# BUTSpeechFIT/VBx

Measured on NVIDIA H100. Metric: x-vectors/sec through 10 VB-HMM EM iters, higher is better.
Workload: dtype f32

## Files before the change

include/vbx_b200.h:

```cpp
#ifndef VBX_B200_H
#define VBX_B200_H

#include <stddef.h>
#include <stdint.h>

#ifdef __cplusplus
extern "C" {
#endif

typedef struct vbx_handle_s *vbx_handle_t;

enum vbx_status {
    VBX_OK = 0,
    VBX_ERR_ARG = -1,
    VBX_ERR_CUDA = -2,
    VBX_ERR_STATE = -3,
    VBX_ERR_NO_DEVICE = -4
};

enum vbx_flag {
    VBX_FLAG_NONFINITE = 1,
    VBX_FLAG_ELBO_DECREASED = 2,
    VBX_FLAG_CONVERGED = 4
};
// ... 161 lines not shown

int vbx_stream_window(vbx_handle_t h, int32_t n, int32_t C, int32_t R, int32_t S_max, int32_t S, const int32_t *slot,
                      const int64_t *blk_off, const int64_t *win_off, const int32_t *blk_lab, const int32_t *n_clusters,
                      const float *blk_fea, double smoothing, const float *ctx_fea, const int32_t *ctx_lab,
                      const int64_t *count, const int32_t *K, const double *n_hist, const double *F_hist, float *fea_out,
                      float *gamma_out, float *pi_out, int32_t *n_states_out, double *prior_n_out, double *prior_F_out,
                      void *stream);
int vbx_stream_commit(vbx_handle_t h, int32_t n, int32_t C, int32_t R, int32_t S_max, const int32_t *slot,
                      const int64_t *blk_off, const int64_t *win_off, const float *blk_fea, const int32_t *first,
                      float *ctx_fea, int32_t *ctx_lab, int64_t *count, int32_t *K, double *n_hist, double *F_hist,
                      int32_t *labels_out, void *stream);

int vbx_stream_enroll_workspace_bytes(vbx_handle_t h, int32_t n, int64_t M, int64_t E, int32_t max_k,
                                      size_t *bytes_out);
int vbx_stream_enroll(vbx_handle_t h, int32_t n, int32_t slots, int32_t C, int32_t R, int32_t S_max,
                      const int32_t *slot, const int64_t *cand_off, const int32_t *cand_k, const float *Phi, double Fa,
                      double Fb, const float *ctx_fea, const int32_t *ctx_lab, const int64_t *count, double *n_hist,
                      double *F_hist, int32_t *named, const double *n_enroll, const double *F_enroll, int64_t E,
                      double threshold, int32_t prior, void *workspace, size_t workspace_bytes, int32_t *assign_out,
                      double *best_llr_out, double *llr_out, double *n_out, double *F_out, void *stream);

int64_t vbx_launch_count(vbx_handle_t h);

enum vbx_kernel_class {
    VBX_K_PROJECT = 0,
    VBX_K_PREPARE = 1,
    VBX_K_RUN_INIT = 2,
    VBX_K_MSTEP = 3,
    VBX_K_SPEAKER_MODEL = 4,
    VBX_K_LOGLIK = 5,
    VBX_K_FWDBWD = 6,
    VBX_K_EXACT64 = 7,
    VBX_K_EM_CONTRACT = 8,
    VBX_N_KERNEL_CLASSES = 9
};
int vbx_get_timings(vbx_handle_t h, double *ms_out, int64_t *count_out, int32_t reset);

#ifdef __cplusplus
}
#endif
#endif
```

vbx_b200/_lib.py:

```python
import ctypes
import os

_HERE = os.path.dirname(os.path.abspath(__file__))
LIB_PATH = os.environ.get('VBX_B200_LIB', os.path.join(_HERE, 'libvbx_b200.so'))

EXPORTS = ['vbx_version', 'vbx_padded_states', 'vbx_padded_states_wide', 'vbx_create', 'vbx_destroy', 'vbx_last_error',
           'vbx_set_option', 'vbx_plan', 'vbx_bind_workspace', 'vbx_prepare_scale',
           'vbx_prepare_project', 'vbx_prepare_xvectors', 'vbx_run', 'vbx_run_per_recording', 'vbx_hard_labels', 'vbx_hard_labels_keep', 'vbx_ahc_workspace_bytes', 'vbx_ahc', 'vbx_launch_count', 'vbx_get_timings', 'vbx_f64_workspace_bytes',
           'vbx_run_f64', 'vbx_plan_f64', 'vbx_forward_backward', 'vbx_attach_comm', 'vbx_elbo_trace', 'vbx_get_gsum',
           'vbx_score', 'vbx_score_overlap', 'vbx_score_jer', 'vbx_link_batch_workspace_bytes', 'vbx_link_batch',
           'vbx_enroll_batch_workspace_bytes', 'vbx_enroll_batch', 'vbx_cohort_stats_batch_workspace_bytes',
           'vbx_cohort_stats_batch', 'vbx_init_turns', 'vbx_combine_workspace_bytes', 'vbx_combine',
           'vbx_init_random', 'vbx_run_prior', 'vbx_run_f64_prior', 'vbx_class_scatter_workspace_bytes',
           'vbx_class_scatter', 'vbx_stream_window', 'vbx_stream_commit', 'vbx_verify_score_workspace_bytes',
           'vbx_verify_score', 'vbx_verify_metrics_workspace_bytes', 'vbx_verify_metrics',
           'vbx_verify_calibrate_workspace_bytes', 'vbx_verify_calibrate', 'vbx_stream_enroll_workspace_bytes',
           'vbx_stream_enroll']

FLAG_NONFINITE, FLAG_ELBO_DECREASED, FLAG_CONVERGED = 1, 2, 4
SCORE_BAD_LABEL, SCORE_BAD_REGION, SCORE_BAD_RECORDING = 1, 2, 4
COMBINE_BAD_LABEL, COMBINE_TOO_MANY_LABELS = 1, 2
LINK_MAX_SPEAKERS = 1 << 29
KERNEL_CLASSES = ['project', 'prepare', 'run_init', 'mstep_partial', 'speaker_model', 'loglik', 'forward_backward', 'exact64', 'em_contract']


class VbxError(RuntimeError):
    pass


_lib = None


def load():
    global _lib
    if _lib is not None:
        return _lib
    if not os.path.exists(LIB_PATH):
        raise VbxError(f'{LIB_PATH} is missing - run `python -c "import __graft_entry__ as g; g.build()"` '
                       '(there is no CPU fallback for the VB-HMM path)')
    lib = ctypes.CDLL(LIB_PATH)
# ... 20 lines not shown
    lib.vbx_bind_workspace.argtypes = [vp, vp, ctypes.c_size_t]
    lib.vbx_prepare_scale.restype = ctypes.c_int
    lib.vbx_prepare_scale.argtypes = [vp, vp, vp, vp, vp]
    lib.vbx_prepare_project.restype = ctypes.c_int
    lib.vbx_prepare_project.argtypes = [vp, vp, i32, vp, vp, vp, vp]
    lib.vbx_ahc_workspace_bytes.restype = ctypes.c_int
    lib.vbx_ahc_workspace_bytes.argtypes = [vp, ctypes.POINTER(ctypes.c_size_t)]
    lib.vbx_ahc.restype = ctypes.c_int
    lib.vbx_ahc.argtypes = [vp, vp, i32, i32, vp, ctypes.c_size_t, vp, vp, vp]
    lib.vbx_hard_labels.restype = ctypes.c_int
    lib.vbx_hard_labels.argtypes = [vp, vp, vp, vp, vp, vp]
    lib.vbx_hard_labels_keep.restype = ctypes.c_int
    lib.vbx_hard_labels_keep.argtypes = [vp, vp, vp, vp, vp, vp, vp, vp]
    lib.vbx_prepare_xvectors.restype = ctypes.c_int
    lib.vbx_prepare_xvectors.argtypes = [vp, vp, i32, vp, vp, vp, vp, vp, vp, vp, vp, vp]
    lib.vbx_run.restype = ctypes.c_int
    lib.vbx_run.argtypes = [vp, vp, vp, vp, vp, vp, dbl, dbl, dbl, i32, dbl, vp, vp, i32, vp, vp, vp, vp]
    lib.vbx_run_per_recording.restype = ctypes.c_int
    lib.vbx_run_per_recording.argtypes = [vp, vp, vp, vp, vp, vp, vp, vp, vp, i32, dbl, vp, vp, i32, vp, vp, vp, vp]
    lib.vbx_run_prior.restype = ctypes.c_int
    lib.vbx_run_prior.argtypes = [vp, vp, vp, vp, vp, vp, vp, vp, vp, i32, dbl, vp, vp, i32, vp, vp, vp, vp, vp, vp]
    lib.vbx_launch_count.restype = i64
    lib.vbx_launch_count.argtypes = [vp]
    lib.vbx_f64_workspace_bytes.restype = ctypes.c_int
    lib.vbx_f64_workspace_bytes.argtypes = [vp, ctypes.POINTER(ctypes.c_size_t)]
    lib.vbx_run_f64.restype = ctypes.c_int
    lib.vbx_run_f64.argtypes = [vp, vp, ctypes.c_size_t, vp, vp, vp, vp, vp, dbl, dbl, dbl, i32, dbl, vp, vp, i32, vp, vp, vp, vp]
    lib.vbx_run_f64_prior.restype = ctypes.c_int
    lib.vbx_run_f64_prior.argtypes = [vp, vp, ctypes.c_size_t, vp, vp, vp, vp, vp, dbl, dbl, dbl, i32, dbl, vp, vp, i32, vp, vp,
                                      vp, vp, vp, vp]
    lib.vbx_forward_backward.restype = ctypes.c_int
    lib.vbx_forward_backward.argtypes = [vp, vp, vp, vp, i32, i32, vp, vp, vp, vp, vp]
    lib.vbx_attach_comm.restype = ctypes.c_int
    lib.vbx_attach_comm.argtypes = [vp, vp, i32, ctypes.c_char_p]
    lib.vbx_elbo_trace.restype = ctypes.c_int
    lib.vbx_elbo_trace.argtypes = [vp, vp, i32, vp, vp]
    lib.vbx_get_gsum.restype = ctypes.c_int
    lib.vbx_get_gsum.argtypes = [vp, vp, vp]
    lib.vbx_score.restype = ctypes.c_int
    lib.vbx_score.argtypes = [vp, i32, vp, vp, vp, vp, vp, vp, vp, vp, vp, i32, vp, vp, vp, vp, vp, i64, vp, vp, vp, vp, vp]
    lib.vbx_score_overlap.restype = ctypes.c_int
    lib.vbx_score_overlap.argtypes = [vp, i32, vp, vp, vp, vp, vp, vp, vp, vp, vp, vp, i32, vp, vp, vp, vp, vp, vp, i64, vp, vp,
                                      vp, vp, vp]
    lib.vbx_score_jer.restype = ctypes.c_int
    lib.vbx_score_jer.argtypes = [vp, i32, vp, vp, vp, vp, vp, vp, vp, vp, vp, vp, i32, vp, vp, vp, vp, vp, vp, i64, vp, vp, vp,
                                  vp, vp, vp, vp]
# ... 67 lines not shown
```

vbx_b200/batch.py:

```python
import ctypes
import os

import numpy as np
import torch

from . import _lib
from ._lib import VbxError


def _ptr(t):
    return ctypes.c_void_p(t.data_ptr()) if t is not None else None


class VbxBatch:

    def __init__(self, lengths, R, n_states, device=None, allocate=True, exact_stop=True, fb_split=0, S_pad=None, f64_only=False):
        if not torch.cuda.is_available():
            raise VbxError('vbx_b200 needs a CUDA device (H100, sm_90); there is no CPU path')
        self.lib = _lib.load()
        self.device = torch.device('cuda', torch.cuda.current_device()) if device is None else torch.device(device)
        if self.device.index is None:
            self.device = torch.device('cuda', torch.cuda.current_device())
        lengths = np.asarray(lengths, dtype=np.int64).reshape(-1)
        self.B = int(lengths.shape[0])
# ... 139 lines not shown
        self._check(self.lib.vbx_init_turns(self._h, *(_ptr(a) for a in arrays), _ptr(gamma), _ptr(pi),
                                            int(dt == torch.float64), self._stream()))

    def init_random(self, rec_keys, seeds, gamma, pi):
        dt = gamma.dtype
        for t, shape, name in ((gamma, (self.N, self.S), 'gamma'), (pi, (self.B, self.S), 'pi')):
            if not (isinstance(t, torch.Tensor) and t.is_cuda and t.dtype == dt and t.is_contiguous()
                    and dt in (torch.float32, torch.float64) and tuple(t.shape) == shape):
                raise ValueError(f'{name}: expected a contiguous float32 or float64 CUDA tensor of shape {shape}, '
                                 'gamma and pi of one type')
        words = []
        for vals, name in ((rec_keys, 'rec_keys'), (seeds, 'seeds')):
            vals = list(vals)
            if len(vals) != self.B or not all(isinstance(v, (int, np.integer)) and 0 <= int(v) < 1 << 64 for v in vals):
                raise ValueError(f'{name}: expected {self.B} integers in [0, 2**64)')
            a = np.array([int(v) for v in vals], dtype=np.uint64).view(np.int64)
            words.append(torch.from_numpy(a).to(self.device))
        self._check(self.lib.vbx_init_random(self._h, _ptr(words[0]), _ptr(words[1]), _ptr(self.n_states), _ptr(gamma),
                                             _ptr(pi), int(dt == torch.float64), self._stream()))

    @property
    def launches(self):
        return int(self.lib.vbx_launch_count(self._h))

    def timings(self, reset=True):
        n = len(_lib.KERNEL_CLASSES)
        ms = (ctypes.c_double * n)()
        cnt = (ctypes.c_int64 * n)()
        self._check(self.lib.vbx_get_timings(self._h, ms, cnt, int(reset)))
        return {k: (ms[i], cnt[i]) for i, k in enumerate(_lib.KERNEL_CLASSES)}

    def _stream(self):
        return ctypes.c_void_p(torch.cuda.current_stream(self.device).cuda_stream)

    def _f32(self, t, shape, name, need_workspace=True):
        if need_workspace and self.workspace is None:
            raise VbxError('no workspace bound (VbxBatch(..., allocate=False) needs bind())')
        if not (isinstance(t, torch.Tensor) and t.is_cuda and t.dtype == torch.float32 and t.is_contiguous()):
            raise ValueError(f'{name}: expected a contiguous float32 CUDA tensor')
        if tuple(t.shape) != tuple(shape):
            raise ValueError(f'{name}: expected shape {tuple(shape)}, got {tuple(t.shape)}')
        return t

    def prepare_scale(self, fea, Phi, out=None):
        self._f32(fea, (self.N, self.R), 'fea')
        self._f32(Phi, (self.R,), 'Phi')
# ... 423 lines not shown
```

vbx_b200/csrc/vbx_capi.cu:

```cuda
#include <dlfcn.h>
#include <nvtx3/nvToolsExt.h>

#include <algorithm>
#include <cmath>
#include <cstdio>
#include <cstring>
#include <initializer_list>
#include <map>
#include <mutex>
#include <numeric>
#include <string>
#include <utility>
#include <vector>

#include "../../include/vbx_b200.h"
#include "vbx_internal.cuh"

bool vbx::allow_dynamic_smem(const void *kernel, int bytes) {
    int dev = 0;
    if (cudaGetDevice(&dev) != cudaSuccess) return false;
    static std::mutex mu;
    static std::map<std::pair<const void *, int>, int> allowed;
    std::lock_guard<std::mutex> lock(mu);
    int &have = allowed[{kernel, dev}];
    if (have >= bytes) return true;
    if (cudaFuncSetAttribute(kernel, cudaFuncAttributeMaxDynamicSharedMemorySize, bytes) != cudaSuccess) return false;
    have = bytes;
    return true;
}

struct vbx_handle_s {
    int device = 0;
    int sms = 0;
    std::string err;
    vbx::Plan plan;
    vbx::Workspace ws;
    bool planned = false, bound = false, prepared = false;
    bool f64_only = false;
    size_t ws_need = 0;
    void *plan_mem = nullptr;
    int opt_fb_spl = 0;
    int opt_fb_classic = 0;
    int opt_fb_ring = 1;
    int opt_projection = 0;
    int opt_timing = 0;
    int opt_gemm = 0;
    int opt_debug_sync = 0;
    int opt_fb_split = 0;
    int opt_exact_stop = 1;
    int64_t launches = 0;
    cudaStream_t hi_stream = nullptr;
    cudaEvent_t ev_fork = nullptr, ev_join = nullptr;
    int opt_graph = 0;
    cudaStream_t graph_stream = nullptr;
    cudaEvent_t ev_g0 = nullptr, ev_g1 = nullptr;
    cudaGraphExec_t graph_exec = nullptr;
    uint64_t graph_key = 0, seen_key = 0;
    int64_t graph_launches = 0;
    bool graph_broken = false;
    void *nccl_comm = nullptr;
    int nccl_ranks = 1;
// ... 355 lines not shown
    pl.R = R;
    pl.S = S;
    pl.exact = h->opt_exact_stop;
    pl.split = split ? 1 : 0;
    pl.em_cluster = vbx::em_contract_cluster(S, R, maxT, split);
    pl.n_frames = n_rec ? offsets_host[n_rec] : 0;
    pl.n_ltiles = (int32_t)lrec.size();
    pl.n_mtiles = (int32_t)mrec.size();
    pl.max_T = maxT;
    pl.offsets = reinterpret_cast<const int64_t *>(base + o_off);
    pl.order = reinterpret_cast<const int32_t *>(base + o_ord);
    pl.ltile_rec = reinterpret_cast<const int32_t *>(base + o_lrec);
    pl.ltile_f0 = reinterpret_cast<const int64_t *>(base + o_lf0);
    pl.mtile_rec = reinterpret_cast<const int32_t *>(base + o_mrec);
    pl.mtile_f0 = reinterpret_cast<const int64_t *>(base + o_mf0);
    pl.mtile_begin = reinterpret_cast<const int32_t *>(base + o_mb);
    pl.n_lrec = (int32_t)lrec_list.size();
    pl.n_lchunks = (int32_t)lchunk_rec.size();
    pl.lrec_list = reinterpret_cast<const int32_t *>(base + o_ll);
    pl.lrec_first = reinterpret_cast<const int32_t *>(base + o_lf);
    pl.lrec_nchunks = reinterpret_cast<const int32_t *>(base + o_ln);
    pl.lchunk_rec = reinterpret_cast<const int32_t *>(base + o_lcr);
    pl.lchunk_idx = reinterpret_cast<const int32_t *>(base + o_lci);
    h->ws_need = carve(pl, nullptr, nullptr);
    h->offsets_host.assign(offsets_host, offsets_host + (n_rec ? n_rec + 1 : 0));
    if (n_rec == 0) h->offsets_host.assign(1, 0);
    h->ahc_need = vbx::ahc_workspace_bytes(h->offsets_host.data(), n_rec, &h->ahc_d_off);
    h->planned = true;
    if (workspace_bytes_out) *workspace_bytes_out = h->ws_need;
    return VBX_OK;
}

int vbx_plan_f64(vbx_handle_t h, const int64_t *offsets_host, int32_t n_rec, int32_t R, int32_t S) {
    if (!h || !offsets_host || n_rec < 0) return fail(h, VBX_ERR_ARG, "vbx_plan_f64: null argument");
    if (R < 1 || S < 1 || S > 3600) return fail(h, VBX_ERR_ARG, "vbx_plan_f64: need R >= 1 and 1 <= S <= 3600");
    if (n_rec > 0 && offsets_host[0] != 0) return fail(h, VBX_ERR_ARG, "vbx_plan_f64: offsets[0] must be 0");
    for (int b = 0; b < n_rec; ++b) {
        const int64_t T = offsets_host[b + 1] - offsets_host[b];
        if (T < 0 || T > (int64_t)1 << 30) return fail(h, VBX_ERR_ARG, "vbx_plan_f64: bad recording length");
    }
    DeviceGuard guard(h->device);
    if (guard.err != cudaSuccess) return cuda_fail(h, guard.err, "cudaSetDevice");
    if (h->plan_mem) {
        cudaFree(h->plan_mem);
        h->plan_mem = nullptr;
    }
    h->planned = h->bound = h->prepared = false;
    cudaError_t e = cudaMalloc(&h->plan_mem, sizeof(int64_t) * (n_rec + 1));
    if (e != cudaSuccess) return cuda_fail(h, e, "cudaMalloc(plan)");
    e = cudaMemcpy(h->plan_mem, offsets_host, sizeof(int64_t) * (n_rec + 1), cudaMemcpyHostToDevice);
    if (e != cudaSuccess) return cuda_fail(h, e, "cudaMemcpy(plan)");
    h->plan = vbx::Plan();
    h->plan.n_rec = n_rec;
    h->plan.R = R;
    h->plan.S = S;
    h->plan.n_frames = n_rec ? offsets_host[n_rec] : 0;
    h->plan.offsets = static_cast<const int64_t *>(h->plan_mem);
    h->offsets_host.assign(offsets_host, offsets_host + n_rec + 1);
    h->ahc_need = 0;
    h->planned = true;
    h->f64_only = true;
    return VBX_OK;
}

int vbx_bind_workspace(vbx_handle_t h, void *workspace, size_t bytes) {
    if (!h) return VBX_ERR_ARG;
    if (!h->planned) return fail(h, VBX_ERR_STATE, "vbx_bind_workspace: call vbx_plan first");
    if (h->f64_only) return fail(h, VBX_ERR_STATE, "vbx_bind_workspace: the plan came from vbx_plan_f64 (float64 entry points only)");
    if (!workspace || bytes < h->ws_need) return fail(h, VBX_ERR_STATE, "vbx_bind_workspace: workspace too small");
    const size_t mis = reinterpret_cast<uintptr_t>(workspace) & 255;
    char *base = static_cast<char *>(workspace) + (mis ? 256 - mis : 0);
    carve(h->plan, base, &h->ws);
    drop_graph(h);
    h->bound = true;
    h->prepared = false;
// ... 185 lines not shown
                    rc = counted(h, h->opt_gemm ? vbx::launch_mstep_partial(pl, h->ws, rho, gamma_io, st)
                                                : vbx::launch_mstep_mma(pl, h->ws, rho, gamma_io, st), "mstep_partial");
                }
                if (rc) return rc;
                {
                    Timed t(h, st, VBX_K_SPEAKER_MODEL);
                    rc = counted(h, vbx::launch_speaker_model(pl, h->ws, Phi, n_states, alpha_io, invL_io, given, st, prior_n,
                                                              prior_F), "speaker_model");
                }
                if (rc) return rc;
                {
                    Timed t(h, st, VBX_K_LOGLIK);
                    rc = counted(h, h->opt_gemm ? vbx::launch_loglik(pl, h->ws, rho, pi_io, n_states, st) : vbx::launch_loglik_mma(pl, h->ws, rho, pi_io, n_states, st), "loglik");
                }
                if (rc) return rc;
            }
            if (fb_hi) {
                cudaEventRecord(h->ev_fork, st);
                cudaStreamWaitEvent(h->hi_stream, h->ev_fork, 0);
            }
            {
                cudaStream_t fs = fb_hi ? h->hi_stream : st;
                Timed t(h, fs, VBX_K_FWDBWD);
                rc = counted(h, vbx::launch_forward_backward(pl, h->ws, rp, gamma_io, pi_io, n_states, Li_out, n_iters_out, flags_out, it, h->opt_fb_spl, h->opt_fb_classic, h->opt_fb_ring, fs), "forward_backward");
            }
            if (fb_hi) {
                cudaEventRecord(h->ev_join, h->hi_stream);
                cudaStreamWaitEvent(st, h->ev_join, 0);
            }
            if (rc) return rc;
        }
        if (rp.hybrid && it > 0) {
            Timed t(h, st, VBX_K_EXACT64);
            rc = counted(h, vbx::launch_exact64_round(pl, h->ws, rp, rho, Phi, gamma_io, pi_io, n_states, alpha_io, invL_io, Li_out,
                                                      n_iters_out, flags_out, st, prior_n, prior_F), "exact64");
            if (rc) return rc;
        }
    }
    return VBX_OK;
    };

    cudaStream_t user = (cudaStream_t)stream;
    const bool want_graph = (h->opt_graph == 1 || (h->opt_graph == 0 && pl.split)) && !h->opt_timing && !h->opt_debug_sync &&
                            !h->graph_broken;
    if (!want_graph) return enqueue(user);
    uint64_t key = 1469598103934665603ull;
    auto mix = [&](uint64_t v) { key = (key ^ v) * 1099511628211ull; };
// ... 872 lines not shown
    if (rc) return rc;
    if (h->nccl_comm && h->nccl_ranks > 1) {
        const int nrc = h->nccl_allreduce(trace_out, trace_out, (size_t)2 * max_iters,  8,  0, h->nccl_comm, st);
        if (nrc != 0) return fail(h, VBX_ERR_CUDA, "vbx_elbo_trace: ncclAllReduce failed with code " + std::to_string(nrc));
    }
    return VBX_OK;
}

int vbx_get_gsum(vbx_handle_t h, double *gsum_out, void *stream) {
    if (!h) return VBX_ERR_ARG;
    if (!h->planned || !h->bound || !h->prepared) return fail(h, VBX_ERR_STATE, "vbx_get_gsum: call vbx_prepare_* first");
    if (h->plan.n_rec == 0) return VBX_OK;
    if (!gsum_out) return fail(h, VBX_ERR_ARG, "vbx_get_gsum: null pointer");
    DeviceGuard guard(h->device);
    if (guard.err != cudaSuccess) return cuda_fail(h, guard.err, "cudaSetDevice");
    const cudaError_t e = cudaMemcpyAsync(gsum_out, h->ws.gsum, sizeof(double) * h->plan.n_rec, cudaMemcpyDeviceToDevice,
                                          (cudaStream_t)stream);
    if (e != cudaSuccess) return cuda_fail(h, e, "vbx_get_gsum");
    return VBX_OK;
}

int64_t vbx_launch_count(vbx_handle_t h) { return h ? h->launches : -1; }

int vbx_get_timings(vbx_handle_t h, double *ms_out, int64_t *count_out, int32_t reset) {
    if (!h) return VBX_ERR_ARG;
    DeviceGuard guard(h->device);
    for (size_t i = 0; i + 1 < h->ev_used; i += 2) {
        cudaError_t e = cudaEventSynchronize(h->ev_pool[i + 1]);
        if (e != cudaSuccess) return cuda_fail(h, e, "cudaEventSynchronize");
        float ms = 0.f;
        e = cudaEventElapsedTime(&ms, h->ev_pool[i], h->ev_pool[i + 1]);
        if (e != cudaSuccess) return cuda_fail(h, e, "cudaEventElapsedTime");
        const int cls = h->ev_class[i / 2];
        h->t_ms[cls] += ms;
        h->t_cnt[cls] += 1;
    }
    h->ev_used = 0;
    h->ev_class.clear();
    for (int c = 0; c < VBX_N_KERNEL_CLASSES; ++c) {
        if (ms_out) ms_out[c] = h->t_ms[c];
        if (count_out) count_out[c] = h->t_cnt[c];
        if (reset) {
            h->t_ms[c] = 0.0;
            h->t_cnt[c] = 0;
        }
    }
// ... 5 lines not shown
```

vbx_b200/csrc/vbx_em_contract.cu:

```cuda
#include <cooperative_groups.h>
#include <math_constants.h>

#include "vbx_internal.cuh"

namespace cg = cooperative_groups;

namespace vbx {

namespace {
constexpr int kSlots = 4;
constexpr int kRows = 8;
constexpr int kHeld = kMTile / kRows / kSlots;
constexpr int kBars = 4;
constexpr int kLD = kMaxR + 4;
constexpr int kRedBytes = 16 * kLD * 4;
constexpr int kRhoBytes = kHeld * kRows * kMaxR * 4;
constexpr int kSmemBytes = kRhoBytes + kRedBytes + (kBars + 1) * 8;

__device__ __forceinline__ uint32_t cluster_addr(uint32_t a, uint32_t rank) {
    uint32_t r;
    asm volatile("mapa.shared::cluster.u32 %0, %1, %2;" : "=r"(r) : "r"(a), "r"(rank));
    return r;
}
__device__ __forceinline__ void st_async(uint32_t addr, float v, uint32_t bar) {
// ... 318 lines not shown
static int em_contract_cluster_t() {
    cudaLaunchConfig_t cfg = {};
    cfg.gridDim = dim3(CL);
    cfg.blockDim = dim3(128);
    cfg.dynamicSmemBytes = kSmemBytes;
    int n = 0;
    if (!allow_dynamic_smem(em_contract_kernel<S_PAD, CL>, kSmemBytes) ||
        cudaOccupancyMaxActiveClusters(&n, em_contract_kernel<S_PAD, CL>, &cfg) != cudaSuccess)
        return (void)cudaGetLastError(), 0;
    return n >= 1 ? CL : 0;
}

int em_contract_cluster(int S, int R, int64_t max_T, bool split) {
    if (split || R != kMaxR || max_T > 2 * kMTile) return 0;
    const bool two = max_T > kMTile;
    switch (S) {
        case 4: return two ? em_contract_cluster_t<4, 8>() : em_contract_cluster_t<4, 4>();
        case 8: return two ? em_contract_cluster_t<8, 8>() : em_contract_cluster_t<8, 4>();
        case 16: return two ? em_contract_cluster_t<16, 8>() : em_contract_cluster_t<16, 4>();
        default: return 0;
    }
}

int launch_em_contract(const Plan &pl, const Workspace &ws, const float *rho, const float *gamma, const float *Phi,
                       const int32_t *n_states, float *alpha_io, float *invL_io, cudaStream_t st) {
    if (pl.n_rec == 0) return 0;
    const int CL = pl.em_cluster;
#define VBX_EMC(S_, CL_)                                                                                                 \
    em_contract_kernel<S_, CL_><<<pl.n_rec * CL_, 128, kSmemBytes, st>>>(pl, ws, rho, gamma, Phi, n_states, alpha_io, invL_io)
    switch (pl.S * 16 + CL) {
        case 4 * 16 + 4: VBX_EMC(4, 4); break;
        case 4 * 16 + 8: VBX_EMC(4, 8); break;
        case 8 * 16 + 4: VBX_EMC(8, 4); break;
        case 8 * 16 + 8: VBX_EMC(8, 8); break;
        case 16 * 16 + 4: VBX_EMC(16, 4); break;
        case 16 * 16 + 8: VBX_EMC(16, 8); break;
        default: return -1;
    }
#undef VBX_EMC
    return cudaGetLastError() == cudaSuccess ? 1 : -1;
}

}
```

vbx_b200/csrc/vbx_internal.cuh:

```cuda
#pragma once
#include <cuda_runtime.h>
#include <stdint.h>

#include <cfloat>
#include <string>
#include <vector>

#define VBX_EPS_TR 1e-8f

namespace vbx {

constexpr int kLTile = 64;
constexpr int kMTile = 512;
constexpr int kLongT = 4096;
constexpr int kChunk = 256;
constexpr int kMaxR = 128;
constexpr int kMaxS = 64;
constexpr int kMaxSWide = 128;
constexpr int kTcMaxD = 2048;

__host__ __device__ inline size_t al(size_t v) { return (v + 255) & ~(size_t)255; }

struct Plan {
    int32_t n_rec = 0, R = 0, S = 0;
// ... 55 lines not shown
    float *scratch = nullptr;
    float *ahat = nullptr, *bhat = nullptr;
    float *socc = nullptr, *sent = nullptr;
    float *tc_scratch = nullptr;
    float *fa_u = nullptr, *fa_lam = nullptr, *fa_exp = nullptr, *astart = nullptr;
    float *bb_v = nullptr, *bb_mu = nullptr, *bb_exp = nullptr, *beta = nullptr;
    float *occp = nullptr, *entp = nullptr;
    RecParams *hp = nullptr;
};

struct RunParams {
    double epsilon;
    int32_t max_iters;
    int32_t hybrid, warm;
};
constexpr double kStopNoiseC = 2.0;
constexpr double kStopGuardMult = 16.0;

bool allow_dynamic_smem(const void *kernel, int bytes);
template <class... Args>
bool allow_dynamic_smem(void (*kernel)(Args...), int bytes) {
    return allow_dynamic_smem(reinterpret_cast<const void *>(kernel), bytes);
}

#ifdef __CUDACC__
template <int N>
struct Vec {
    float v[N];
};
template <int N>
__device__ __forceinline__ Vec<N> ld_vec(const float *p);
template <>
__device__ __forceinline__ Vec<1> ld_vec<1>(const float *p) {
    Vec<1> r;
    r.v[0] = *p;
    return r;
}
template <>
__device__ __forceinline__ Vec<2> ld_vec<2>(const float *p) {
    float2 t = *reinterpret_cast<const float2 *>(p);
    Vec<2> r;
    r.v[0] = t.x;
    r.v[1] = t.y;
    return r;
}
template <>
// ... 194 lines not shown

__device__ __forceinline__ double as_norm(double l, const double *mean_i, const double *std_i, int64_t i,
                                          const double *mean_j, const double *std_j, int64_t j) {
    return 0.5 * ((l - mean_i[i]) / std_i[i] + (l - mean_j[j]) / std_j[j]);
}

#endif

int launch_prepare_scale(const Plan &pl, const Workspace &ws, const float *fea, const float *Phi, float *rho,
                         cudaStream_t st);
int launch_project_ffma(const Plan &pl, const float *X, int D, const float *V, float *rho, cudaStream_t st);
int launch_g_from_rho(const Plan &pl, const Workspace &ws, const float *rho, const float *Phi, cudaStream_t st);
int launch_run_init(const Plan &pl, const Workspace &ws, const float *gamma, const int32_t *n_states, double *Li,
                    int32_t *n_iters, int32_t *flags, int max_iters, double Fa, double Fb, double loopP,
                    const double *Fa_v, const double *Fb_v, const double *loopP_v, cudaStream_t st);
int launch_mstep_partial(const Plan &pl, const Workspace &ws, const float *rho, const float *gamma, cudaStream_t st);
int launch_speaker_model(const Plan &pl, const Workspace &ws, const float *Phi,
                         const int32_t *n_states, float *alpha_io, float *invL_io, bool from_given,
                         cudaStream_t st, const double *prior_n = nullptr, const double *prior_F = nullptr);
int launch_loglik(const Plan &pl, const Workspace &ws, const float *rho, const float *pi, const int32_t *n_states,
                  cudaStream_t st);
int launch_forward_backward(const Plan &pl, const Workspace &ws, const RunParams &rp, float *gamma, float *pi,
                            const int32_t *n_states, double *Li, int32_t *n_iters, int32_t *flags, int iter,
                            int spl, int classic, int ring, cudaStream_t st);
int launch_elbo_trace(const Plan &pl, const double *Li, int max_iters, double *out, cudaStream_t st);
int launch_forward_backward_split(const Plan &pl, const Workspace &ws, const RunParams &rp, float *gamma, float *pi,
                                  const int32_t *n_states, int spl, cudaStream_t st);
int launch_forward_backward_long(const Plan &pl, const Workspace &ws, const RunParams &rp, float *gamma, float *pi,
                                 const int32_t *n_states, cudaStream_t st);
int launch_mstep_mma(const Plan &pl, const Workspace &ws, const float *rho, const float *gamma, cudaStream_t st);
int launch_loglik_mma(const Plan &pl, const Workspace &ws, const float *rho, const float *pi, const int32_t *n_states,
                      cudaStream_t st);
int em_contract_cluster(int S, int R, int64_t max_T, bool split);
int launch_em_contract(const Plan &pl, const Workspace &ws, const float *rho, const float *gamma, const float *Phi,
                       const int32_t *n_states, float *alpha_io, float *invL_io, cudaStream_t st);
int launch_snapshot(const Plan &pl, const Workspace &ws, const float *gamma, const float *pi, int iter, cudaStream_t st);
int launch_exact64_round(const Plan &pl, const Workspace &ws, const RunParams &rp, const float *rho, const float *Phi,
                         float *gamma, float *pi, const int32_t *n_states, float *alpha_io, float *invL_io, double *Li,
                         int32_t *n_iters, int32_t *flags, cudaStream_t st, const double *prior_n = nullptr,
                         const double *prior_F = nullptr);
size_t f64_workspace_bytes(const Plan &pl);
int launch_run_f64(const Plan &pl, void *workspace, const double *fea, const double *Phi, double *gamma, double *pi,
                   const int32_t *n_states, double Fa, double Fb, double loopP, int max_iters, double epsilon,
                   double *alpha_io, double *invL_io, int warm, double *Li, int32_t *n_iters, int32_t *flags,
                   cudaStream_t st, const double *prior_n = nullptr, const double *prior_F = nullptr);
int launch_hard_labels(const Plan &pl, const float *gamma, const int32_t *n_states, int32_t *first, int32_t *second,
                       cudaStream_t st);
int launch_hard_labels_keep(const Plan &pl, const float *gamma, const int32_t *n_states, const int32_t *keep,
                            int32_t *first, int32_t *second, double *mass, cudaStream_t st);
int launch_init_turns(const Plan &pl, const int64_t *seg, const int64_t *spk_off, const int64_t *turn_off,
                      const int64_t *turn_lo, const int64_t *turn_hi, const int64_t *turn_cum, const double *smoothing,
                      void *gamma, void *pi, bool f64, cudaStream_t st);
int launch_init_random(const Plan &pl, const uint64_t *rec_key, const uint64_t *seed, const int32_t *n_states,
                       void *gamma, void *pi, bool f64, cudaStream_t st);
int launch_fb_dense(const double *lls, const double *tr, const double *ip, int T, int S, double *post, double *tll,
                    double *lfw, double *lbw, cudaStream_t st);
// ... 116 lines not shown
```

vbx_b200/csrc/vbx_kernels.cu:

```cuda
#include <math_constants.h>

#include "vbx_internal.cuh"

namespace vbx {

__device__ __forceinline__ void cp_async16(void *smem, const void *gmem) {
    unsigned s = static_cast<unsigned>(__cvta_generic_to_shared(smem));
    asm volatile("cp.async.cg.shared.global [%0], [%1], 16;\n" ::"r"(s), "l"(gmem));
}
__device__ __forceinline__ void cp_async_wait_all() {
    asm volatile("cp.async.commit_group;\n" ::);
    asm volatile("cp.async.wait_group 0;\n" ::: "memory");
}

template <int LANES>
__device__ __forceinline__ float group_max(float v) {
#pragma unroll
    for (int off = LANES / 2; off > 0; off >>= 1) v = fmaxf(v, __shfl_xor_sync(0xffffffffu, v, off));
    return v;
}
__device__ __forceinline__ double warp_sum_d(double v) {
#pragma unroll
    for (int off = 16; off > 0; off >>= 1) v += __shfl_xor_sync(0xffffffffu, v, off);
    return v;
// ... 1512 lines not shown
            else
                bstage(u, st, rb, true);
        }
    }

    double pn[SPL];
    float loc = 0.f;
#pragma unroll
    for (int k = 0; k < SPL; ++k) {
        pn[k] = (double)g0[k] + (double)Q * (double)pi[k] * enter[k];
        loc += (float)pn[k];
    }
    const float tot = group_sum<LPR>(loc);
    if (live) {
#pragma unroll
        for (int k = 0; k < SPL; ++k) {
            const int s = l * SPL + k;
            pi_io[(int64_t)rec * S_PAD + s] = (float)(pn[k] / (double)tot);
            ws.occ[(int64_t)rec * S_PAD + s] = (float)occ[k];
        }
    }
}

constexpr int64_t kRingMaxT = 2048;

template <int S_PAD, int SPL>
static int launch_fb_t(const Plan &pl, const Workspace &ws, const RunParams &rp, float *gamma, float *pi,
                       const int32_t *n_states, bool classic, bool ring, cudaStream_t st) {
    constexpr int RPW = 32 / (S_PAD / SPL);
    const int warps = (pl.n_rec + RPW - 1) / RPW;
    const int blocks = (warps + 3) / 4;
    if (classic) {
        forward_backward_kernel<S_PAD, SPL><<<blocks, 128, 0, st>>>(pl, ws, rp, gamma, pi, n_states);
    } else if (ring && pl.max_T <= kRingMaxT) {
        constexpr int smem = FbRing<S_PAD, SPL>::kSmemBytes;
        if (!allow_dynamic_smem(forward_backward_ring_kernel<S_PAD, SPL>, smem)) return -1;
        forward_backward_ring_kernel<S_PAD, SPL><<<blocks, 128, smem, st>>>(pl, ws, rp, gamma, pi, n_states);
    } else {
        forward_backward_la_kernel<S_PAD, SPL><<<blocks, 128, 0, st>>>(pl, ws, rp, gamma, pi, n_states);
    }
    return cudaGetLastError() == cudaSuccess ? 1 : -1;
}

__global__ void __launch_bounds__(128) elbo_kernel(Plan pl, Workspace ws, RunParams rp, double *Li, int32_t *n_iters,
                                                   int32_t *flags, int iter) {
    const int rec = blockIdx.x;
    if (!ws.active[rec]) return;
    const int tid = threadIdx.x, lane = tid & 31, warp = tid >> 5;
    const int64_t f0 = pl.offsets[rec];
    const int T = (int)(pl.offsets[rec + 1] - f0);
    const float *rs = ws.rsigma + f0;
    const float *mx = ws.rowmax + f0;
    double acc = 0.0;
    for (int t = tid; t < T; t += 128) acc += (double)mx[t] - log((double)rs[t]);
    acc = warp_sum_d(acc);
    __shared__ double part[4];
// ... 49 lines not shown
    __shared__ double ss[256], cs[256];
    ss[tid] = s;
    cs[tid] = c;
    __syncthreads();
    for (int off = 128; off > 0; off >>= 1) {
        if (tid < off) {
            ss[tid] += ss[tid + off];
            cs[tid] += cs[tid + off];
        }
        __syncthreads();
    }
    if (tid == 0) {
        out[it] = ss[0];
        out[max_iters + it] = cs[0];
    }
}
int launch_elbo_trace(const Plan &pl, const double *Li, int max_iters, double *out, cudaStream_t st) {
    elbo_trace_kernel<<<max_iters, 256, 0, st>>>(pl.n_rec, Li, max_iters, out);
    return cudaGetLastError() == cudaSuccess ? 1 : -1;
}

int launch_forward_backward(const Plan &pl, const Workspace &ws, const RunParams &rp, float *gamma, float *pi,
                            const int32_t *n_states, double *Li, int32_t *n_iters, int32_t *flags, int iter,
                            int spl, int classic, int ring, cudaStream_t st) {
    if (pl.n_rec == 0) return 0;
    if (pl.split) {
        const int rs = launch_forward_backward_split(pl, ws, rp, gamma, pi, n_states, spl, st);
        if (rs < 0) return rs;
        elbo_kernel<<<pl.n_rec, 128, 0, st>>>(pl, ws, rp, Li, n_iters, flags, iter);
        return cudaGetLastError() == cudaSuccess ? rs + 1 : -1;
    }
    int rc = -1;
#define VBX_FB(S_, L_) rc = launch_fb_t<S_, L_>(pl, ws, rp, gamma, pi, n_states, classic != 0, ring != 0, st)
    const int S = pl.S;
    if (spl == 0) spl = (S >= 16) ? 2 : 1;
    if (S == 64 && spl < 2) spl = 2;
    if (spl > S) spl = S;
    switch (S) {
        case 4:
            if (spl == 1) VBX_FB(4, 1);
            else if (spl == 2) VBX_FB(4, 2);
            else VBX_FB(4, 4);
            break;
        case 8:
            if (spl == 1) VBX_FB(8, 1);
            else if (spl == 2) VBX_FB(8, 2);
            else VBX_FB(8, 4);
            break;
        case 16:
            if (spl == 1) VBX_FB(16, 1);
            else if (spl == 2) VBX_FB(16, 2);
            else VBX_FB(16, 4);
            break;
        case 32:
            if (spl == 1) VBX_FB(32, 1);
            else if (spl == 2) VBX_FB(32, 2);
// ... 18 lines not shown
```

Measured before the change: 201.9 million.

## Add shared-memory-free forward-backward kernel that co-resides with EM contraction

Adds a forward-backward variant that keeps its checkpoints in the gamma output buffer instead of dynamic shared memory. It is chosen when an occupancy check shows one of its CTAs fits on an SM beside the resident em_contract CTAs, so the two stages can overlap across streams. It also sets the max-shared carveout preference on the new kernel and on the ELBO kernel. The cost is more global-memory traffic for checkpoint reloads, plus a host-side occupancy heuristic that may misjudge residency.

```diff
diff --git a/include/vbx_b200.h b/include/vbx_b200.h
--- a/include/vbx_b200.h
+++ b/include/vbx_b200.h
@@ -207,6 +207,8 @@
 
 int64_t vbx_launch_count(vbx_handle_t h);
 
+int vbx_plan_property(vbx_handle_t h, const char *name, int32_t *value_out);
+
 enum vbx_kernel_class {
     VBX_K_PROJECT = 0,
     VBX_K_PREPARE = 1,
diff --git a/vbx_b200/_lib.py b/vbx_b200/_lib.py
--- a/vbx_b200/_lib.py
+++ b/vbx_b200/_lib.py
@@ -15,7 +15,7 @@
            'vbx_class_scatter', 'vbx_stream_window', 'vbx_stream_commit', 'vbx_verify_score_workspace_bytes',
            'vbx_verify_score', 'vbx_verify_metrics_workspace_bytes', 'vbx_verify_metrics',
            'vbx_verify_calibrate_workspace_bytes', 'vbx_verify_calibrate', 'vbx_stream_enroll_workspace_bytes',
-           'vbx_stream_enroll']
+           'vbx_stream_enroll', 'vbx_plan_property']
 
 FLAG_NONFINITE, FLAG_ELBO_DECREASED, FLAG_CONVERGED = 1, 2, 4
 SCORE_BAD_LABEL, SCORE_BAD_REGION, SCORE_BAD_RECORDING = 1, 2, 4
@@ -82,6 +82,8 @@
     lib.vbx_run_prior.argtypes = [vp, vp, vp, vp, vp, vp, vp, vp, vp, i32, dbl, vp, vp, i32, vp, vp, vp, vp, vp, vp]
     lib.vbx_launch_count.restype = i64
     lib.vbx_launch_count.argtypes = [vp]
+    lib.vbx_plan_property.restype = ctypes.c_int
+    lib.vbx_plan_property.argtypes = [vp, ctypes.c_char_p, ctypes.POINTER(i32)]
     lib.vbx_f64_workspace_bytes.restype = ctypes.c_int
     lib.vbx_f64_workspace_bytes.argtypes = [vp, ctypes.POINTER(ctypes.c_size_t)]
     lib.vbx_run_f64.restype = ctypes.c_int
diff --git a/vbx_b200/batch.py b/vbx_b200/batch.py
--- a/vbx_b200/batch.py
+++ b/vbx_b200/batch.py
@@ -185,6 +185,11 @@
     @property
     def launches(self):
         return int(self.lib.vbx_launch_count(self._h))
+
+    def plan_property(self, name):
+        v = ctypes.c_int32()
+        self._check(self.lib.vbx_plan_property(self._h, name.encode(), ctypes.byref(v)))
+        return int(v.value)
 
     def timings(self, reset=True):
         n = len(_lib.KERNEL_CLASSES)
diff --git a/vbx_b200/csrc/vbx_capi.cu b/vbx_b200/csrc/vbx_capi.cu
--- a/vbx_b200/csrc/vbx_capi.cu
+++ b/vbx_b200/csrc/vbx_capi.cu
@@ -9,6 +9,7 @@
 #include <map>
 #include <mutex>
 #include <numeric>
+#include <set>
 #include <string>
 #include <utility>
 #include <vector>
@@ -29,6 +30,19 @@
     return true;
 }
 
+bool vbx::prefer_max_shared(const void *kernel) {
+    int dev = 0;
+    if (cudaGetDevice(&dev) != cudaSuccess) return false;
+    static std::mutex mu;
+    static std::set<std::pair<const void *, int>> done;
+    std::lock_guard<std::mutex> lock(mu);
+    if (done.count({kernel, dev})) return true;
+    if (cudaFuncSetAttribute(kernel, cudaFuncAttributePreferredSharedMemoryCarveout, cudaSharedmemCarveoutMaxShared) != cudaSuccess)
+        return false;
+    done.insert({kernel, dev});
+    return true;
+}
+
 struct vbx_handle_s {
     int device = 0;
     int sms = 0;
@@ -37,6 +51,7 @@
     vbx::Workspace ws;
     bool planned = false, bound = false, prepared = false;
     bool f64_only = false;
+    bool fb_beside = false;
     size_t ws_need = 0;
     void *plan_mem = nullptr;
     int opt_fb_spl = 0;
@@ -438,6 +453,7 @@
     pl.lrec_nchunks = reinterpret_cast<const int32_t *>(base + o_ln);
     pl.lchunk_rec = reinterpret_cast<const int32_t *>(base + o_lcr);
     pl.lchunk_idx = reinterpret_cast<const int32_t *>(base + o_lci);
+    h->fb_beside = vbx::fb_beside_fits(pl, h->sms);
     h->ws_need = carve(pl, nullptr, nullptr);
     h->offsets_host.assign(offsets_host, offsets_host + (n_rec ? n_rec + 1 : 0));
     if (n_rec == 0) h->offsets_host.assign(1, 0);
@@ -467,6 +483,7 @@
     e = cudaMemcpy(h->plan_mem, offsets_host, sizeof(int64_t) * (n_rec + 1), cudaMemcpyHostToDevice);
     if (e != cudaSuccess) return cuda_fail(h, e, "cudaMemcpy(plan)");
     h->plan = vbx::Plan();
+    h->fb_beside = false;
     h->plan.n_rec = n_rec;
     h->plan.R = R;
     h->plan.S = S;
@@ -698,7 +715,7 @@
             {
                 cudaStream_t fs = fb_hi ? h->hi_stream : st;
                 Timed t(h, fs, VBX_K_FWDBWD);
-                rc = counted(h, vbx::launch_forward_backward(pl, h->ws, rp, gamma_io, pi_io, n_states, Li_out, n_iters_out, flags_out, it, h->opt_fb_spl, h->opt_fb_classic, h->opt_fb_ring, fs), "forward_backward");
+                rc = counted(h, vbx::launch_forward_backward(pl, h->ws, rp, gamma_io, pi_io, n_states, Li_out, n_iters_out, flags_out, it, h->opt_fb_spl, h->opt_fb_classic, h->opt_fb_ring, h->fb_beside, fs), "forward_backward");
             }
             if (fb_hi) {
                 cudaEventRecord(h->ev_join, h->hi_stream);
@@ -1617,6 +1634,17 @@
 
 int64_t vbx_launch_count(vbx_handle_t h) { return h ? h->launches : -1; }
 
+int vbx_plan_property(vbx_handle_t h, const char *name, int32_t *value_out) {
+    if (!h || !name || !value_out) return VBX_ERR_ARG;
+    if (!h->planned) return fail(h, VBX_ERR_STATE, "vbx_plan_property: call vbx_plan first");
+    const vbx::Plan &pl = h->plan;
+    if (!strcmp(name, "split")) *value_out = pl.split;
+    else if (!strcmp(name, "em_cluster")) *value_out = pl.em_cluster;
+    else if (!strcmp(name, "fb_beside")) *value_out = h->fb_beside ? 1 : 0;
+    else return fail(h, VBX_ERR_ARG, std::string("vbx_plan_property: unknown property ") + name);
+    return VBX_OK;
+}
+
 int vbx_get_timings(vbx_handle_t h, double *ms_out, int64_t *count_out, int32_t reset) {
     if (!h) return VBX_ERR_ARG;
     DeviceGuard guard(h->device);
diff --git a/vbx_b200/csrc/vbx_em_contract.cu b/vbx_b200/csrc/vbx_em_contract.cu
--- a/vbx_b200/csrc/vbx_em_contract.cu
+++ b/vbx_b200/csrc/vbx_em_contract.cu
@@ -364,7 +364,39 @@
     }
 }
 
-int launch_em_contract(const Plan &pl, const Workspace &ws, const float *rho, const float *gamma, const float *Phi,
+bool em_contract_leaves_room(int S, int CL, const void *kernel, int threads) {
+    const void *emc = nullptr;
+    switch (S * 16 + CL) {
+        case 4 * 16 + 4: emc = reinterpret_cast<const void *>(em_contract_kernel<4, 4>); break;
+        case 4 * 16 + 8: emc = reinterpret_cast<const void *>(em_contract_kernel<4, 8>); break;
+        case 8 * 16 + 4: emc = reinterpret_cast<const void *>(em_contract_kernel<8, 4>); break;
+        case 8 * 16 + 8: emc = reinterpret_cast<const void *>(em_contract_kernel<8, 8>); break;
+        case 16 * 16 + 4: emc = reinterpret_cast<const void *>(em_contract_kernel<16, 4>); break;
+        case 16 * 16 + 8: emc = reinterpret_cast<const void *>(em_contract_kernel<16, 8>); break;
+        default: return false;
+    }
+    int dev = 0, n = 0, regs = 0, smem = 0, reserved = 0, max_threads = 0, max_ctas = 0;
+    cudaFuncAttributes ea, ka;
+    if (cudaGetDevice(&dev) != cudaSuccess || cudaFuncGetAttributes(&ea, emc) != cudaSuccess ||
+        cudaFuncGetAttributes(&ka, kernel) != cudaSuccess ||
+        cudaOccupancyMaxActiveBlocksPerMultiprocessor(&n, emc, 128, kSmemBytes) != cudaSuccess ||
+        cudaDeviceGetAttribute(&regs, cudaDevAttrMaxRegistersPerMultiprocessor, dev) != cudaSuccess ||
+        cudaDeviceGetAttribute(&smem, cudaDevAttrMaxSharedMemoryPerMultiprocessor, dev) != cudaSuccess ||
+        cudaDeviceGetAttribute(&reserved, cudaDevAttrReservedSharedMemoryPerBlock, dev) != cudaSuccess ||
+        cudaDeviceGetAttribute(&max_threads, cudaDevAttrMaxThreadsPerMultiProcessor, dev) != cudaSuccess ||
+        cudaDeviceGetAttribute(&max_ctas, cudaDevAttrMaxBlocksPerMultiprocessor, dev) != cudaSuccess)
+        return (void)cudaGetLastError(), false;
+    auto cta_regs = [](const cudaFuncAttributes &a, int nthreads) {
+        return (nthreads + 31) / 32 * ((a.numRegs * 32 + 255) / 256 * 256);
+    };
+    auto cta_smem = [&](const cudaFuncAttributes &a, int dynamic) {
+        return ((int)a.sharedSizeBytes + dynamic + reserved + 127) / 128 * 128;
+    };
+    return n * cta_regs(ea, 128) + cta_regs(ka, threads) <= regs && n * cta_smem(ea, kSmemBytes) + cta_smem(ka, 0) <= smem &&
+           n * 128 + threads <= max_threads && n + 1 <= max_ctas;
+}
+
+int launch_em_contract(const Plan &pl,const Workspace &ws, const float *rho, const float *gamma, const float *Phi,
                        const int32_t *n_states, float *alpha_io, float *invL_io, cudaStream_t st) {
     if (pl.n_rec == 0) return 0;
     const int CL = pl.em_cluster;
diff --git a/vbx_b200/csrc/vbx_internal.cuh b/vbx_b200/csrc/vbx_internal.cuh
--- a/vbx_b200/csrc/vbx_internal.cuh
+++ b/vbx_b200/csrc/vbx_internal.cuh
@@ -101,6 +101,11 @@
 bool allow_dynamic_smem(void (*kernel)(Args...), int bytes) {
     return allow_dynamic_smem(reinterpret_cast<const void *>(kernel), bytes);
 }
+bool prefer_max_shared(const void *kernel);
+template <class... Args>
+bool prefer_max_shared(void (*kernel)(Args...)) {
+    return prefer_max_shared(reinterpret_cast<const void *>(kernel));
+}
 
 #ifdef __CUDACC__
 template <int N>
@@ -341,7 +346,7 @@
                   cudaStream_t st);
 int launch_forward_backward(const Plan &pl, const Workspace &ws, const RunParams &rp, float *gamma, float *pi,
                             const int32_t *n_states, double *Li, int32_t *n_iters, int32_t *flags, int iter,
-                            int spl, int classic, int ring, cudaStream_t st);
+                            int spl, int classic, int ring, bool beside, cudaStream_t st);
 int launch_elbo_trace(const Plan &pl, const double *Li, int max_iters, double *out, cudaStream_t st);
 int launch_forward_backward_split(const Plan &pl, const Workspace &ws, const RunParams &rp, float *gamma, float *pi,
                                   const int32_t *n_states, int spl, cudaStream_t st);
@@ -351,6 +356,8 @@
 int launch_loglik_mma(const Plan &pl, const Workspace &ws, const float *rho, const float *pi, const int32_t *n_states,
                       cudaStream_t st);
 int em_contract_cluster(int S, int R, int64_t max_T, bool split);
+bool em_contract_leaves_room(int S, int CL, const void *kernel, int threads);
+bool fb_beside_fits(const Plan &pl, int sms);
 int launch_em_contract(const Plan &pl, const Workspace &ws, const float *rho, const float *gamma, const float *Phi,
                        const int32_t *n_states, float *alpha_io, float *invL_io, cudaStream_t st);
 int launch_snapshot(const Plan &pl, const Workspace &ws, const float *gamma, const float *pi, int iter, cudaStream_t st);
diff --git a/vbx_b200/csrc/vbx_kernels.cu b/vbx_b200/csrc/vbx_kernels.cu
--- a/vbx_b200/csrc/vbx_kernels.cu
+++ b/vbx_b200/csrc/vbx_kernels.cu
@@ -1558,16 +1558,313 @@
     }
 }
 
+template <int S_PAD, int SPL>
+__global__ void __launch_bounds__(128) forward_backward_beside_kernel(Plan pl, Workspace ws, RunParams rp, float *gamma,
+                                                                      float *pi_io, const int32_t *__restrict__ n_states) {
+    constexpr int LPR = S_PAD / SPL;
+    constexpr int PF = (SPL == 4) ? 10 : (SPL == 2 ? 24 : 32);
+    constexpr int F = FbRing<S_PAD, SPL>::F;
+    const int lane = threadIdx.x & 31;
+    const int warp_global = blockIdx.x * 4 + (threadIdx.x >> 5);
+    const int g = lane / LPR, l = lane % LPR;
+    const int slot = warp_global * (32 / LPR) + g;
+    int rec = -1;
+    if (slot < pl.n_rec) rec = pl.order[slot];
+    const bool live = rec >= 0 && ws.active[rec] != 0 && pl.lrec_nchunks[rec] == 0;
+    int64_t f0 = 0;
+    int T = 0;
+    if (live) {
+        f0 = pl.offsets[rec];
+        T = (int)(pl.offsets[rec + 1] - f0);
+    }
+    int Tmax = T, Tmin = live ? T : 0x7fffffff;
+#pragma unroll
+    for (int off = 16; off > 0; off >>= 1) {
+        Tmax = max(Tmax, __shfl_xor_sync(0xffffffffu, Tmax, off));
+        Tmin = min(Tmin, __shfl_xor_sync(0xffffffffu, Tmin, off));
+    }
+    if (Tmax == 0) return;
+    const int Tlast = max(T - 1, 0);
+    const int ns = live ? (n_states ? n_states[rec] : S_PAD) : 0;
+    const float P = rec >= 0 ? ws.hp[rec].loopP : 0.f, Q = 1.f - P;
+
+    float pi[SPL], w[SPL];
+#pragma unroll
+    for (int k = 0; k < SPL; ++k) {
+        const int s = l * SPL + k;
+        const bool sl = live && s < ns;
+        pi[k] = sl ? pi_io[(int64_t)rec * S_PAD + s] : 0.f;
+        w[k] = sl ? fmaf(Q, pi[k], VBX_EPS_TR) : 0.f;
+    }
+    const float *pp = ws.p + f0 * S_PAD + l * SPL;
+    float *ga = live ? gamma + f0 * S_PAD + l * SPL : ws.scratch + l * SPL;
+    float *rs = live ? ws.rsigma + f0 : ws.scratch + kMaxS;
+    const int64_t gstr = live ? S_PAD : 0;
+    const int rstr = live ? 1 : 0;
+    const float *gg = ga - l * SPL;
+
+    float alast[SPL];
+    {
+        FwdState<SPL> fs;
+        const Vec<SPL> p1 = ldg_vec<SPL>(pp + (int64_t)min(1, Tlast) * S_PAD);
+        fwd_init<SPL, LPR>(fs, ldg_vec<SPL>(pp), p1, pi, w, l, live, ns, alast);
+        st_vec<SPL>(ga, alast);
+        if (l == 0) rs[0] = fs.rs1;
+        auto fstep = [&](const int j, const Vec<SPL> &ps, const Vec<SPL> &pn, const bool check) {
+            const int s = j + 1, kb = T - 1 - s;
+            if (kb >= F && kb % F == 0) {
+                sto_vec<SPL>(ga + s * gstr, fs.y);
+                if (l == 0) {
+                    const float sc[4] = {fs.Yc, fs.q, fs.c, fs.rn};
+                    sto_vec<4>(ga + (s + 1) * gstr, sc);
+                    sto_vec<1>(ga + (s + 2) * gstr, &fs.rs1);
+                }
+            }
+            float an[SPL];
+            const float rsig = fwd_step<SPL, LPR>(fs, ps, pn, w, P, an);
+            const bool act = !check || s < T;
+#pragma unroll
+            for (int k = 0; k < SPL; ++k) alast[k] = act ? an[k] : alast[k];
+            if (act) {
+                if (s == T - 1) sto_vec<SPL>(ga + s * gstr, an);
+                if (l == 0) rs[s * rstr] = rsig;
+            }
+        };
+        Vec<SPL> bufA[PF], bufB[PF];
+        Vec<SPL> ps = p1;
+        auto fchunk = [&](const int j0, Vec<SPL>(&cur)[PF], Vec<SPL>(&nxt)[PF], const bool check) {
+#pragma unroll
+            for (int i = 0; i < PF; ++i) nxt[i] = ldo_vec<SPL>(pp + (int64_t)min(j0 + PF + i + 2, Tlast) * S_PAD);
+#pragma unroll
+            for (int i = 0; i < PF; ++i) {
+                fstep(j0 + i, ps, cur[i], check);
+                ps = cur[i];
+            }
+        };
+#pragma unroll
+        for (int i = 0; i < PF; ++i) bufA[i] = ldg_vec<SPL>(pp + (int64_t)min(i + 2, Tlast) * S_PAD);
+        int j0 = 0;
+        for (; j0 + 2 * PF <= Tmin - 1; j0 += 2 * PF) {
+            fchunk(j0, bufA, bufB, false);
+            fchunk(j0 + PF, bufB, bufA, false);
+        }
+        for (; j0 < Tmax - 1; j0 += 2 * PF) {
+            fchunk(j0, bufA, bufB, true);
+            fchunk(j0 + PF, bufB, bufA, true);
+        }
+    }
+    __syncwarp();
+
+    float g0[SPL], occf[SPL], entf[SPL];
+    double enter[SPL], occ[SPL];
+#pragma unroll
+    for (int k = 0; k < SPL; ++k) {
+        g0[k] = alast[k];
+        occ[k] = (double)alast[k];
+        enter[k] = 0.0;
+        occf[k] = 0.f;
+        entf[k] = 0.f;
+    }
+    {
+        float b[SPL], kap[SPL];
+        float dprev = 1.f, e = 0.f, f;
+        {
+            const Vec<SPL> pl1 = ldo_vec<SPL>(pp + (int64_t)Tlast * S_PAD);
+            const float rl1 = ldo_vec<1>(rs + Tlast * rstr).v[0];
+            float locf = 0.f;
+#pragma unroll
+            for (int k = 0; k < SPL; ++k) {
+                b[k] = 1.f;
+                kap[k] = pl1.v[k] * rl1;
+                locf = fmaf(w[k], kap[k], locf);
+            }
+            f = group_sum<LPR>(locf);
+        }
+        auto bstep = [&](const int ii, const Vec<SPL> &a, const Vec<SPL> &pt, const float rt, const bool check) {
+            const int t = T - 2 - ii;
+            float v[SPL], kapn[SPL], loce = 0.f, locf = 0.f;
+#pragma unroll
+            for (int k = 0; k < SPL; ++k) {
+                v[k] = kap[k] * b[k];
+                kapn[k] = pt.v[k] * rt;
+                const float wk = w[k] * kapn[k];
+                loce = fmaf(wk, v[k], loce);
+                locf += wk;
+            }
+            const float en = group_sum<LPR>(loce);
+            const float fn = group_sum<LPR>(locf);
+            const float d = fmaf(P, e, dprev * f);
+            float gn[SPL], bn[SPL], gs = 0.f;
+#pragma unroll
+            for (int k = 0; k < SPL; ++k) {
+                bn[k] = fmaf(P, v[k], d);
+                gn[k] = a.v[k] * bn[k];
+                gs += gn[k];
+            }
+            {
+                const float sc = rcp_fast(group_sum<LPR>(gs));
+#pragma unroll
+                for (int k = 0; k < SPL; ++k) gn[k] *= sc;
+            }
+            if (!check) {
+#pragma unroll
+                for (int k = 0; k < SPL; ++k) {
+                    g0[k] = gn[k];
+                    occf[k] += gn[k];
+                    entf[k] += v[k];
+                }
+                sto_vec<SPL>(ga + t * gstr, gn);
+            } else {
+                const bool act = t >= 0;
+#pragma unroll
+                for (int k = 0; k < SPL; ++k) {
+                    g0[k] = act ? gn[k] : g0[k];
+                    occf[k] += act ? gn[k] : 0.f;
+                    entf[k] += act ? v[k] : 0.f;
+                }
+                if (act) sto_vec<SPL>(ga + t * gstr, gn);
+            }
+#pragma unroll
+            for (int k = 0; k < SPL; ++k) {
+                b[k] = bn[k];
+                kap[k] = kapn[k];
+            }
+            dprev = d;
+            e = en;
+            f = fn;
+        };
+        struct Stage {
+            Vec<SPL> p[F];
+            float r[F];
+            Vec<SPL> cy, q0, q1;
+            Vec<4> c4;
+            float crs;
+        };
+        auto load_stage = [&](const int u, Stage &sg) {
+            const int lo = T - 1 - (u + 1) * F, lc = max(lo, 0), z = min(max(-lo, 0), F - 1);
+#pragma unroll
+            for (int i = 0; i < F; ++i) {
+                sg.p[i] = ldo_vec<SPL>(pp + (int64_t)min(max(lo + i, 0), Tlast) * S_PAD);
+                sg.r[i] = ldo_vec<1>(rs + min(max(lo + F - 1 - i, 0), Tlast) * rstr).v[0];
+            }
+            sg.q0 = ldo_vec<SPL>(pp + (int64_t)min(max(lo + z, 0), Tlast) * S_PAD);
+            sg.q1 = ldo_vec<SPL>(pp + (int64_t)min(max(lo + min(z + 1, F - 1), 0), Tlast) * S_PAD);
+            sg.cy = ldo_vec<SPL>(ga + min(lc, Tlast) * gstr);
+            sg.c4 = ldo_vec<4>(gg + min(lc + 1, Tlast) * gstr);
+            sg.crs = ldo_vec<1>(gg + min(lc + 2, Tlast) * gstr).v[0];
+        };
+        auto bstage = [&](const int u, const Stage &cur, Stage &nxt, const bool check) {
+            load_stage(u + 1, nxt);
+            const int lo = T - 1 - (u + 1) * F;
+            FwdState<SPL> fs, f1;
+            {
+                float a0[SPL];
+                fwd_init<SPL, LPR>(f1, cur.q0, cur.q1, pi, w, l, live, ns, a0);
+                const bool ck = lo >= 1;
+#pragma unroll
+                for (int k = 0; k < SPL; ++k) {
+                    fs.y[k] = ck ? cur.cy.v[k] : f1.y[k];
+                    f1.y[k] = a0[k];
+                }
+                fs.Yc = ck ? cur.c4.v[0] : f1.Yc;
+                fs.q = ck ? cur.c4.v[1] : f1.q;
+                fs.c = ck ? cur.c4.v[2] : f1.c;
+                fs.rn = ck ? cur.c4.v[3] : f1.rn;
+                fs.rs1 = ck ? cur.crs : f1.rs1;
+            }
+            Vec<SPL> a[F];
+#pragma unroll
+            for (int i = 0; i < F; ++i) {
+                const int s = lo + i;
+                FwdState<SPL> nx = fs;
+                fwd_step<SPL, LPR>(nx, cur.p[i], cur.p[min(i + 1, F - 1)], w, P, a[i].v);
+                if (s >= 1) fs = nx;
+#pragma unroll
+                for (int k = 0; k < SPL; ++k) a[i].v[k] = s == 0 ? f1.y[k] : a[i].v[k];
+            }
+#pragma unroll
+            for (int i = 0; i < F; ++i) bstep(u * F + i, a[F - 1 - i], cur.p[F - 1 - i], cur.r[i], check);
+#pragma unroll
+            for (int k = 0; k < SPL; ++k) {
+                occ[k] += (double)occf[k];
+                enter[k] += (double)entf[k];
+                occf[k] = 0.f;
+                entf[k] = 0.f;
+            }
+        };
+        Stage sA, sB;
+        load_stage(0, sA);
+        const int nb = (Tmax - 1 + F - 1) / F;
+        int u = 0;
+        for (; u + 2 <= nb && (u + 2) * F <= Tmin - 1; u += 2) {
+            bstage(u, sA, sB, false);
+            bstage(u + 1, sB, sA, false);
+        }
+        for (; u < nb; u += 2) {
+            bstage(u, sA, sB, true);
+            if (u + 1 < nb) bstage(u + 1, sB, sA, true);
+        }
+    }
+
+    double pn[SPL];
+    float loc = 0.f;
+#pragma unroll
+    for (int k = 0; k < SPL; ++k) {
+        pn[k] = (double)g0[k] + (double)Q * (double)pi[k] * enter[k];
+        loc += (float)pn[k];
+    }
+    const float tot = group_sum<LPR>(loc);
+    if (live) {
+#pragma unroll
+        for (int k = 0; k < SPL; ++k) {
+            const int s = l * SPL + k;
+            pi_io[(int64_t)rec * S_PAD + s] = (float)(pn[k] / (double)tot);
+            ws.occ[(int64_t)rec * S_PAD + s] = (float)occ[k];
+        }
+    }
+}
+
 constexpr int64_t kRingMaxT = 2048;
+
+__global__ void __launch_bounds__(128) elbo_kernel(Plan pl, Workspace ws, RunParams rp, double *Li, int32_t *n_iters,
+                                                   int32_t *flags, int iter);
+
+template <int S_PAD, int SPL>
+constexpr bool kHasBeside = S_PAD <= 16 && SPL == (S_PAD >= 16 ? 2 : 1);
+
+template <int S_PAD, int SPL>
+static int fb_blocks(const Plan &pl) {
+    constexpr int RPW = 32 / (S_PAD / SPL);
+    const int warps = (pl.n_rec + RPW - 1) / RPW;
+    return (warps + 3) / 4;
+}
+
+template <int S_PAD, int SPL>
+static bool fb_beside_fits_t(const Plan &pl, int sms) {
+    return fb_blocks<S_PAD, SPL>(pl) <= sms &&
+           em_contract_leaves_room(S_PAD, pl.em_cluster, reinterpret_cast<const void *>(forward_backward_beside_kernel<S_PAD, SPL>), 128);
+}
+bool fb_beside_fits(const Plan &pl, int sms) {
+    if (!pl.em_cluster || pl.split || pl.n_rec < 1024 || pl.max_T > kRingMaxT) return false;
+    switch (pl.S) {
+        case 4: return fb_beside_fits_t<4, 1>(pl, sms);
+        case 8: return fb_beside_fits_t<8, 1>(pl, sms);
+        case 16: return fb_beside_fits_t<16, 2>(pl, sms);
+        default: return false;
+    }
+}
 
 template <int S_PAD, int SPL>
 static int launch_fb_t(const Plan &pl, const Workspace &ws, const RunParams &rp, float *gamma, float *pi,
-                       const int32_t *n_states, bool classic, bool ring, cudaStream_t st) {
-    constexpr int RPW = 32 / (S_PAD / SPL);
-    const int warps = (pl.n_rec + RPW - 1) / RPW;
-    const int blocks = (warps + 3) / 4;
+                       const int32_t *n_states, bool classic, bool ring, bool beside, cudaStream_t st) {
+    const int blocks = fb_blocks<S_PAD, SPL>(pl);
     if (classic) {
         forward_backward_kernel<S_PAD, SPL><<<blocks, 128, 0, st>>>(pl, ws, rp, gamma, pi, n_states);
+    } else if (kHasBeside<S_PAD, SPL> && ring && beside) {
+        if constexpr (kHasBeside<S_PAD, SPL>) {
+            if (!prefer_max_shared(forward_backward_beside_kernel<S_PAD, SPL>) || !prefer_max_shared(elbo_kernel)) return -1;
+            forward_backward_beside_kernel<S_PAD, SPL><<<blocks, 128, 0, st>>>(pl, ws, rp, gamma, pi, n_states);
+        }
     } else if (ring && pl.max_T <= kRingMaxT) {
         constexpr int smem = FbRing<S_PAD, SPL>::kSmemBytes;
         if (!allow_dynamic_smem(forward_backward_ring_kernel<S_PAD, SPL>, smem)) return -1;
@@ -1663,7 +1960,7 @@
 
 int launch_forward_backward(const Plan &pl, const Workspace &ws, const RunParams &rp, float *gamma, float *pi,
                             const int32_t *n_states, double *Li, int32_t *n_iters, int32_t *flags, int iter,
-                            int spl, int classic, int ring, cudaStream_t st) {
+                            int spl, int classic, int ring, bool beside, cudaStream_t st) {
     if (pl.n_rec == 0) return 0;
     if (pl.split) {
         const int rs = launch_forward_backward_split(pl, ws, rp, gamma, pi, n_states, spl, st);
@@ -1672,7 +1969,7 @@
         return cudaGetLastError() == cudaSuccess ? rs + 1 : -1;
     }
     int rc = -1;
-#define VBX_FB(S_, L_) rc = launch_fb_t<S_, L_>(pl, ws, rp, gamma, pi, n_states, classic != 0, ring != 0, st)
+#define VBX_FB(S_, L_) rc = launch_fb_t<S_, L_>(pl, ws, rp, gamma, pi, n_states, classic != 0, ring != 0, beside, st)
     const int S = pl.S;
     if (spl == 0) spl = (S >= 16) ? 2 : 1;
     if (S == 64 && spl < 2) spl = 2;
```

Result: slower. 190.3 million (median of 6 runs) (-5.8%).
